# DreamOneX/yet-another-bpe

Measured on AMD Instinct MI355X. Metric: merges_per_sec, higher is better.
Workload: dtype u16

## Files before the change

### yet-another-bpe_amd/csrc/yabpe.hip

```cpp
#include <hip/hip_runtime.h>
#include <dlfcn.h>
#include <rccl/rccl.h>

#include <algorithm>
#include <cstdarg>
#include <cstddef>
#include <cstdio>
#include <cstring>
#include <map>
#include <mutex>
#include <string>
#include <vector>

#include "../../include/yabpe.h"
#include "yabpe_kernels.h"
#include "yabpe_aux_kernels.h"
#include "yabpe_devmem.h"
#include "yabpe_pretok_kernels.h"
#include "yabpe_encode_kernels.h"
#include "yabpe_dropout_kernels.h"
#include "yabpe_decode_kernels.h"
#include "yabpe_layout_kernels.h"
#include "yabpe_replay_kernels.h"
#include "yabpe_pool_kernels.h"
// ... 134 lines not shown
    uint8_t *dec_text = nullptr;
    unsigned long long *dec_doc = nullptr;
    yabpe_decode_stats_t dec_stats{};
    hipEvent_t dec_ev[7] = {};
    uint32_t *lay_buf[7] = {};
    yabpe_layout_stats_t lay_stats{};
    hipEvent_t lay_ev[4] = {};
    yabpe_resume_stats_t resume_stats{};
    bool have_pool = false;
    PoolView wpool{};
    uint64_t wpool_arena_cap = 0, wpool_n = 0, wpool_bytes = 0;
    yabpe_pool_stats_t wpool_stats{};
    hipEvent_t wpool_ev[4] = {};
    unsigned long long *scratch64 = nullptr;
    unsigned long long *blk_stats = nullptr;
    uint32_t blk_used = 0;
    bool split_mode = false;
    uint32_t kmax_now = 1;
    std::vector<float> ev_scan_us;
    unsigned long long *sig = nullptr;
    uint32_t sig_stride = 0;
    unsigned long long *blk_read = nullptr;
    uint64_t scan_skip_launches = 0;
    uint64_t piece_tag = 0;
    bool sig_valid = false;
    uint32_t sig_built_at = 0;
    uint64_t sig_tokens_at_build = 0;
    uint64_t sig_builds = 0;
    CandState *cand_state = nullptr;
    uint32_t cand_built_at = 0;
    unsigned long long cand_best_at_build = 0;
    uint32_t *sel_ticket = nullptr;
    unsigned long long *cand = nullptr;
    bool use_cand = false;
    uint64_t cand_rebuilds = 0, cand_rescans = 0;
    double cand_margin = 0.2;
    uint32_t cand_n_at_build = 0;
    bool pending = false;
    uint64_t fused_launches = 0;
    int rank = 0, n_ranks = 1;
    bool multi = false;
    ncclComm_t comm = nullptr;
    yabpe_allgather_fn ag_fn = nullptr;
    void *ag_user = nullptr;
    unsigned long long *xsmall = nullptr;
    uint8_t *xsend = nullptr, *xrecv = nullptr;
    uint64_t exchange_growths = 0;
    uint64_t exchange_max_records = 0;
    uint32_t xcap = 0;
    uint64_t xstride = 0;
    uint32_t xeff = 0;
    uint64_t xeff_sum = 0;
    uint32_t xseen[4] = {0, 0, 0, 0};
    uint64_t exchanges = 0;
    bool p2p = false;
    uint8_t *p2p_area = nullptr;
    std::vector<uint8_t *> p2p_peer;
    uint64_t p2p_half = 0, p2p_flags_off = 0, p2p_seq = 0, p2p_stride = 0;
    uint32_t p2p_cap = 0;
    hipEvent_t p2p_e0 = nullptr, p2p_e1 = nullptr;
    bool p2p_pending = false;
    int id_bits = 16;
    bool id_bits_fixed = false;
    uint32_t *tiles32 = nullptr, *tiles32_alt = nullptr, *long_tok32 = nullptr;
    uint32_t tiles32_alt_cap = 0;
    PairTable32 table32{};
// ... 69 lines not shown

int fill_u16(yabpe_ctx *c, uint16_t *p, uint64_t n, uint16_t v) {
    if (!n) return 0;
    uint64_t th = (n + 7) / 8;
    hipLaunchKernelGGL(k_fill_u16, dim3(cdiv64(th, 256)), dim3(256), 0, c->stream, p, (unsigned long long)n, v);
    HIPCHK(c, hipGetLastError());
    return 0;
}
int fill_u32(yabpe_ctx *c, uint32_t *p, uint64_t n, uint32_t v) {
    if (!n) return 0;
    hipLaunchKernelGGL(k_fill_u32, dim3(cdiv64(n, 256)), dim3(256), 0, c->stream, p, (unsigned long long)n, v);
    HIPCHK(c, hipGetLastError());
    return 0;
}

int state_pull(yabpe_ctx *c) {
    HIPCHK(c, hipMemcpyAsync(c->st_host, c->st, sizeof(DevState), hipMemcpyDeviceToHost, c->stream));
    HIPCHK(c, hipStreamSynchronize(c->stream));
    return 0;
}
int state_push(yabpe_ctx *c) {
    HIPCHK(c, hipMemcpyAsync(c->st, c->st_host, sizeof(DevState), hipMemcpyHostToDevice, c->stream));
    HIPCHK(c, hipStreamSynchronize(c->stream));
    return 0;
}

void table_free(PairTable &t) {
    dfree(t.keys);
    dfree(t.cnt);
    t.keys = nullptr;
    t.cnt = nullptr;
    t.cand_cs = nullptr;
    t.cand_list = nullptr;
    t.cand_T = 0;
    t.sink_rec = nullptr;
    t.sink_hdr = nullptr;
    t.sink_cap = 0;
}

int table_alloc(yabpe_ctx *c, PairTable &t, uint64_t cap, unsigned long long *entries_ctr) {
    TRY(dmalloc(c, &t.keys, cap));
    TRY(dmalloc(c, &t.cnt, cap));
    t.cap = (uint32_t)cap;
    t.max_probe = c->multi ? (uint32_t)cap : (uint32_t)std::min<uint64_t>(cap, 2048);
    t.sink_rec = nullptr;
    t.sink_hdr = nullptr;
    t.sink_cap = 0;
    t.entries = entries_ctr;
    t.cand_cs = nullptr;
    t.cand_list = nullptr;
    t.cand_T = 0;
    HIPCHK(c, hipMemsetAsync(t.keys, 0xFF, cap * sizeof(uint32_t), c->stream));
    HIPCHK(c, hipMemsetAsync(t.cnt, 0, cap * sizeof(unsigned long long), c->stream));
    return 0;
}

int cand_attach(yabpe_ctx *c) {
    c->use_cand = false;
    PairTable &t = c->table;
    t.cand_cs = nullptr;
    t.cand_list = nullptr;
    if (!optv(c, "cand_argmax", 1)) return 0;
    if (!c->sel_ticket) {
        TRY(dmalloc(c, &c->sel_ticket, TICKET_WORDS));
        HIPCHK(c, hipMemsetAsync(c->sel_ticket, 0, TICKET_WORDS * 4, c->stream));
    }
    if (!c->cand_state) {
        TRY(dmalloc(c, &c->cand_state, 1));
        TRY(dmalloc(c, &c->cand, CAND_CAP));
    }
    return 0;
}

int cand_rebuild(yabpe_ctx *c, unsigned long long best_count) {
    c->use_cand = false;
    c->table.cand_cs = nullptr;
    c->table.cand_list = nullptr;
    if (!optv(c, "cand_argmax", 1) || !c->cand_state || best_count < (unsigned long long)optv(c, "cand_min_count", 16)) return 0;
    const uint32_t target = (uint32_t)std::max<int64_t>(64, optv(c, "cand_target", 768));
    const uint32_t grid = (uint32_t)std::min<uint64_t>(1024, std::max<uint64_t>(1, c->table_cap / (BLOCK * 8)));
    CandState h{};
    for (int attempt = 0; attempt < 12; ++attempt) {
        unsigned long long margin = (unsigned long long)((double)best_count * c->cand_margin);
        if (margin < 1) margin = 1;
        h = CandState{best_count - std::min(margin, best_count - 1), 0u, 0u, 0u, 0u};
        HIPCHK(c, hipMemcpyAsync(c->cand_state, &h, sizeof h, hipMemcpyHostToDevice, c->stream));
        PairTable t = c->table;
        t.cand_list = c->cand;
        t.cand_cs = c->cand_state;
        t.cand_T = h.T;
        {
            CandParams P{t, c->tt.rec, c->partials, c->st, c->cand_state, nullptr, SelectParams{}};
            hipLaunchKernelGGL(k_cand_rebuild, dim3(grid), dim3(BLOCK), 0, c->stream, P);
        }
        HIPCHK(c, hipGetLastError());
        HIPCHK(c, hipMemcpyAsync(&h, c->cand_state, sizeof h, hipMemcpyDeviceToHost, c->stream));
        HIPCHK(c, hipStreamSynchronize(c->stream));
        c->cand_rebuilds++;
        if ((h.overflow || h.n > target) && margin > 1) {
            c->cand_margin *= 0.5;
            continue;
        }
        break;
    }
    if (h.n < target / 8) c->cand_margin = std::min((double)optv(c, "cand_margin_max_pct", 60) / 100.0, c->cand_margin * 2.0);
    c->use_cand = !h.overflow && h.n < CAND_CAP / 2;
    c->cand_n_at_build = h.n;
    if (c->use_cand) {
        c->table.cand_cs = c->cand_state;
        c->table.cand_list = c->cand;
        c->table.cand_T = h.T;
    }
    return 0;
}

uint32_t count_grid(yabpe_ctx *c) {
    return count_grid_rule(c->n_tiles, (uint32_t)c->n_cu, (uint32_t)c->apply_occ, optv(c, "apply_blocks", OPT_UNSET));
}

int fold_stats(yabpe_ctx *c) {
    FoldParams F{c->st, c->blk_stats, std::max(c->blk_used, 1u)};
    hipLaunchKernelGGL(k_fold_stats, dim3(1), dim3(BLOCK), 0, c->stream, F);
    HIPCHK(c, hipGetLastError());
    c->blk_used = 0;
    return 0;
}

int comm_allgather(yabpe_ctx *c, const void *send, void *recv, uint64_t nbytes) {
    if (c->comm) {
        NCCLCHK(c, rccl()->AllGather(send, recv, nbytes, ncclUint8, c->comm, c->stream));
        return 0;
    }
    if (!c->ag_fn) return fail(c, YABPE_E_COMM, "no transport attached");
    HIPCHK(c, hipStreamSynchronize(c->stream));
    int rc = c->ag_fn(c->ag_user, send, recv, nbytes);
    if (rc != 0) return fail(c, YABPE_E_COMM, "custom all-gather transport failed (%d)", rc);
    return 0;
}

int comm_max(yabpe_ctx *c, unsigned long long v, unsigned long long *out);

int exchange_table(yabpe_ctx *c, PairTable lt, uint64_t lcap, PairTable t) {
    unsigned long long *d_cnt = &c->scratch64[8];
// ... 737 lines not shown
    for (auto &e : c->enc_ev)
        if (e) (void)hipEventDestroy(e);
    yabpe_decode_free(c);
    dfree(c->dec_ent); dfree(c->dec_pool);
    for (auto &e : c->dec_ev)
        if (e) (void)hipEventDestroy(e);
    yabpe_layout_free(c);
    for (auto &e : c->lay_ev)
        if (e) (void)hipEventDestroy(e);
    yabpe_pool_clear(c);
    for (auto &e : c->wpool_ev)
        if (e) (void)hipEventDestroy(e);
    dfree(c->pt_cls);
    dfree(c->pt_cls5);
    yabpe_normalize_free(c);
    dfree(c->nfc_prop); dfree(c->nfc_decomp); dfree(c->nfc_pairs);
    for (auto &e : c->norm_ev)
        if (e) (void)hipEventDestroy(e);
    free_corpus(c);
    id32_free_corpus(c);
    dfree(c->partials32);
    dfree(c->cand32_state);
    dfree(c->cand32_list);
    free_records(c);
    dfree(c->tt.pool); dfree(c->tt.off); dfree(c->tt.len); dfree(c->tt.rec); dfree(c->tt.vset);
    dfree(c->partials);
    dfree(c->st);
    dfree(c->scratch64);
    dfree(c->blk_stats);
    dfree(c->blk_read);
    dfree(c->cand_state);
    dfree(c->sel_ticket);
    dfree(c->cand);
    dfree(c->xsend);
    dfree(c->xrecv);
    dfree(c->xsmall);
    p2p_close(c);
    if (c->p2p_e0) (void)hipEventDestroy(c->p2p_e0);
    if (c->p2p_e1) (void)hipEventDestroy(c->p2p_e1);
    if (c->comm && rccl()) (void)rccl()->CommDestroy(c->comm);
    if (c->st_host) (void)hipHostFree(c->st_host);
    for (auto &e : c->events) {
        (void)hipEventDestroy(e.e0);
        (void)hipEventDestroy(e.e1);
        (void)hipEventDestroy(e.e2);
    }
    if (c->stream) (void)hipStreamDestroy(c->stream);
    delete c;
}

int yabpe_set_option(yabpe_ctx *c, const char *name, int64_t value) {
    if (!c || !name) return YABPE_E_INVALID;
    if (strcmp(name, "id_bits") == 0) {
        if (value != 16 && value != 32) return fail(c, YABPE_E_INVALID, "option id_bits is %lld: 16 or 32", (long long)value);
        if (c->id_bits_fixed && value != c->id_bits)
            return fail(c, YABPE_E_INVALID, "option id_bits cannot change after yabpe_set_vocab (it is %d)", c->id_bits);
        if (value == 32 && c->multi) return fail(c, YABPE_E_INVALID, "id_bits = 32 is single-device: this context has a communicator attached");
        if (!c->id_bits_fixed) c->id_bits = (int)value;
    }
    c->opt[name] = value;
    return YABPE_OK;
}

int yabpe_set_vocab(yabpe_ctx *c, const uint8_t *tok_bytes, const uint32_t *tok_off, uint32_t n_tokens) {
    if (!c) return YABPE_E_INVALID;
    HIPCHK(c, hipSetDevice(c->device));
// ... 2740 lines not shown
```

### yet-another-bpe_amd/csrc/yabpe_kernels.h

```cpp
#pragma once
#include <hip/hip_runtime.h>
#include <stdint.h>

#include <type_traits>

#include "limit_logic.h"
#include "load_logic.h"
#include "steal_logic.h"
#include "tile_logic.h"
#include "train_rules.h"

namespace yb {

constexpr int CAP = 1024;
constexpr int LMAX = 64;
constexpr int SPAN = CAP - LMAX + 1;
constexpr uint32_t EMPTY = 0xFFFFFFFFu;
constexpr uint32_t PADPAD = (YB_PAD << 16) | YB_PAD;
constexpr int LONG_CH = 1024;
constexpr int SIG_ROWS = 512;
constexpr int SIG_ROWS_LOG2 = 9;
constexpr int SIG_TILES = 8;
constexpr int MAX_LISTS_PROF = 4096;
constexpr int SCAN_CHUNK = 256;
constexpr int SCAN_KT_MAX = 4;

enum : uint32_t { HALT_NONE = 0, HALT_TABLE_FULL = 1, HALT_POOL_FULL = 2, HALT_VOCAB_FULL = 3, HALT_DELTA_FULL = 4, HALT_RESCAN = 5, HALT_COMM = 6 };

struct BatchMerge {
    uint32_t a, b, c, is_new;
};
struct DevState {
    uint32_t iter;
    uint32_t done;
    uint32_t halt;
    uint32_t halt_req;
    uint32_t a, b, c;
    uint32_t c_is_new;
    uint32_t n_tokens;
    uint32_t pool_used;
// ... 13 lines not shown
    uint32_t n_batch;
    uint32_t n_select;
    BatchMerge batch[KMAX];
    const uint32_t *tok_len;
    uint32_t max_token_bytes;
    uint32_t pad_limit;
};

struct DeltaHdr {
    unsigned long long count;
    unsigned long long halt;
};
struct DeltaRec {
    uint32_t key, pad;
    long long delta;
};

constexpr uint32_t CAND_CAP = 1u << 16;
struct CandState {
    unsigned long long T;
    uint32_t n, overflow;
    uint32_t n_seen;
    uint32_t pad;
};

struct PairTable {
    uint32_t *keys;
    unsigned long long *cnt;
    uint32_t cap;
    uint32_t max_probe;
    unsigned long long *entries;
    CandState *cand_cs;
    unsigned long long *cand_list;
    unsigned long long cand_T;
    DeltaRec *sink_rec;
    DeltaHdr *sink_hdr;
    uint32_t sink_cap;
};
__device__ __forceinline__ uint32_t hash32(uint32_t k);
__device__ __forceinline__ uint32_t pt_home(const PairTable &t, uint32_t key) {
    return (uint32_t)(((unsigned long long)hash32(key) * t.cap) >> 32);
}
__device__ __forceinline__ uint32_t pt_next(const PairTable &t, uint32_t s) { return s + 1 == t.cap ? 0u : s + 1; }

struct Best {
    unsigned long long cnt;
    uint32_t rk;
    uint32_t key;
    uint32_t slot;
    uint32_t pad;
};

__device__ __forceinline__ void best_store_coherent(Best *p, const Best &b) {
    unsigned long long *q = reinterpret_cast<unsigned long long *>(p);
    __hip_atomic_store(q + 0, b.cnt, __ATOMIC_RELAXED, __HIP_MEMORY_SCOPE_AGENT);
    __hip_atomic_store(q + 1, ((unsigned long long)b.key << 32) | b.rk, __ATOMIC_RELAXED, __HIP_MEMORY_SCOPE_AGENT);
    __hip_atomic_store(q + 2, (unsigned long long)b.slot, __ATOMIC_RELAXED, __HIP_MEMORY_SCOPE_AGENT);
}
__device__ __forceinline__ Best best_load_coherent(const Best *p) {
    unsigned long long *q = reinterpret_cast<unsigned long long *>(const_cast<Best *>(p));
    const unsigned long long a = __hip_atomic_load(q + 0, __ATOMIC_RELAXED, __HIP_MEMORY_SCOPE_AGENT);
    const unsigned long long b = __hip_atomic_load(q + 1, __ATOMIC_RELAXED, __HIP_MEMORY_SCOPE_AGENT);
    const unsigned long long c = __hip_atomic_load(q + 2, __ATOMIC_RELAXED, __HIP_MEMORY_SCOPE_AGENT);
    return Best{a, (uint32_t)b, (uint32_t)(b >> 32), (uint32_t)c, 0u};
}

// ... 38 lines not shown
    const SigHash H = sig_hash(key);
    return SigProbe{sig + (size_t)H.row * stride, H.mask};
}

__device__ __forceinline__ void vm_drain() { __builtin_amdgcn_s_waitcnt(0x0F70); }

__device__ __forceinline__ void wave_sync() {
    __builtin_amdgcn_fence(__ATOMIC_RELEASE, "wavefront");
    __builtin_amdgcn_wave_barrier();
    __builtin_amdgcn_fence(__ATOMIC_ACQUIRE, "wavefront");
}

__device__ __forceinline__ unsigned long long lanemask_lt(int lane) { return (1ull << lane) - 1ull; }
__device__ __forceinline__ uint32_t bits_below_lane(unsigned long long m) {
    return __builtin_amdgcn_mbcnt_hi((uint32_t)(m >> 32), __builtin_amdgcn_mbcnt_lo((uint32_t)m, 0u));
}

__device__ __forceinline__ uint32_t wave_inclusive_sum(uint32_t x) {
    x += (uint32_t)__builtin_amdgcn_update_dpp(0, (int)x, 0x111, 0xf, 0xf, true);
    x += (uint32_t)__builtin_amdgcn_update_dpp(0, (int)x, 0x112, 0xf, 0xf, true);
    x += (uint32_t)__builtin_amdgcn_update_dpp(0, (int)x, 0x114, 0xf, 0xf, true);
    x += (uint32_t)__builtin_amdgcn_update_dpp(0, (int)x, 0x118, 0xf, 0xf, true);
    x += (uint32_t)__builtin_amdgcn_update_dpp(0, (int)x, 0x142, 0xa, 0xf, false);
    x += (uint32_t)__builtin_amdgcn_update_dpp(0, (int)x, 0x143, 0xc, 0xf, false);
    return x;
}

__device__ __forceinline__ void st_coherent(unsigned long long *p, unsigned long long v) { __hip_atomic_store(p, v, __ATOMIC_RELAXED, __HIP_MEMORY_SCOPE_AGENT); }
__device__ __forceinline__ void st_coherent(uint32_t *p, uint32_t v) { __hip_atomic_store(p, v, __ATOMIC_RELAXED, __HIP_MEMORY_SCOPE_AGENT); }
__device__ __forceinline__ unsigned long long ld_coherent(const unsigned long long *p) { return __hip_atomic_load(const_cast<unsigned long long *>(p), __ATOMIC_RELAXED, __HIP_MEMORY_SCOPE_AGENT); }
__device__ __forceinline__ uint32_t ld_coherent(const uint32_t *p) { return __hip_atomic_load(const_cast<uint32_t *>(p), __ATOMIC_RELAXED, __HIP_MEMORY_SCOPE_AGENT); }

__device__ __forceinline__ void cand_note(const PairTable &t, uint32_t s, uint32_t key, unsigned long long old, unsigned long long now) {
    if ((long long)now < (long long)t.cand_T || (long long)old >= (long long)t.cand_T || (long long)now <= 0) return;
    const uint32_t idx = atomicAdd(&t.cand_cs->n, 1u);
    if (idx < CAND_CAP)
        st_coherent(&t.cand_list[idx], (unsigned long long)s | ((unsigned long long)key << 32));
    else
        st_coherent(&t.cand_cs->overflow, 1u);
}
__device__ __forceinline__ unsigned long long *pt_count_ptr(const PairTable &t, unsigned long long entry) { return &t.cnt[(uint32_t)entry]; }
__device__ __forceinline__ void gt_bump(const PairTable &t, uint32_t s, uint32_t key, long long d) {
    if (d > 0 && t.cand_list) {
        const unsigned long long old = atomicAdd(&t.cnt[s], (unsigned long long)d);
        cand_note(t, s, key, old, old + (unsigned long long)d);
    } else {
        atomicAdd(&t.cnt[s], (unsigned long long)d);
    }
}

__device__ __forceinline__ void sink_append(const PairTable &t, uint32_t key, long long d) {
    const unsigned long long idx = atomicAdd(&t.sink_hdr->count, 1ull);
    if (idx < t.sink_cap) t.sink_rec[idx] = DeltaRec{key, 0u, d};
}
__device__ __forceinline__ void gt_add_from(const PairTable &t, DevState *st, uint32_t key, long long d, uint32_t s, uint32_t *inserted) {
    if (t.sink_rec) {
        sink_append(t, key, d);
        return;
    }
    for (uint32_t probe = 0; probe < t.max_probe; ++probe) {
        uint32_t k = __hip_atomic_load(&t.keys[s], __ATOMIC_RELAXED, __HIP_MEMORY_SCOPE_AGENT);
        if (k == EMPTY) {
            const uint32_t lim = st->max_token_bytes;
            if (lim != 0u) {
                const uint32_t *len = st->tok_len;
                if (!yb_pair_fits(len[key >> 16], len[key & 0xffffu], lim)) return;
            }
// ... 1685 lines not shown
    __syncthreads();
    if ((tid & 63) == 0) {
        s_b[tid >> 6] = best;
        if (fa | ff) {
            atomicAdd(&s_fold[0], fa);
            atomicAdd(&s_fold[1], ff);
        }
    }
    __syncthreads();
    YB_SEL_STAMP(2);
    if (tid == 0) {
        for (int w = 1; w < WPB; ++w)
            if (best_gt(s_b[w], best)) best = s_b[w];
        s_flag = sel_stop(P, S, s_fold[0], s_fold[1], best.cnt);
        s_m.cnt = best.cnt;
        s_m.key = best.key;
        s_m.slot = best.slot;
    }
    __syncthreads();
    if (s_flag) return;
    YB_SEL_STAMP(3);
    if (tid < 2) {
        const TokRec r = P.tt.rec[tid ? s_m.key & 0xffffu : s_m.key >> 16];
        if (tid) { s_m.hy = r.hash; s_m.ly = r.len; s_m.py = r.pre8; } else { s_m.hx = r.hash; s_m.lx = r.len; s_m.px = r.pre8; }
    }
    __syncthreads();
    YB_SEL_STAMP(4);
    if (tid < 64) commit_merge(P, S, s_m);
    YB_SEL_STAMP(7);
}

__device__ __forceinline__ void select_eval(const SelectParams &P, WinEnt *s_win) {
    __shared__ AccEnt s_acc[KMAX];
    __shared__ __attribute__((aligned(16))) uint32_t s_hset[2 * WIN];
    __shared__ unsigned long long s_red[WPB], s_fold[2];
    __shared__ uint32_t s_nwin;
    struct TopEnt { unsigned long long cnt; uint32_t key, win; };
    __shared__ unsigned long long s_lim[2];
    __shared__ uint32_t s_flags[2];
    unsigned long long *s_pk = reinterpret_cast<unsigned long long *>(s_hset);
    __shared__ TopEnt s_top[KMAX];
    static_assert(BLOCK == 2 * WIN, "two threads rank one window entry");
    constexpr uint32_t HSET = 2 * WIN;
    DevState *st = P.st;
    const int tid = threadIdx.x;
    const int lane = tid & 63;
    YB_SEL_STAMP(1);
    unsigned long long e[4], cn[4];
#pragma unroll
    for (int k = 0; k < 4; ++k) e[k] = ld_coherent(&P.table.cand_list[tid + k * BLOCK]);
    const uint32_t n_list = min(ld_coherent(&P.cs->n), CAND_CAP);
    const uint32_t kmax = min(st->kmax, (uint32_t)KMAX);
    SelState S{};
    if (tid == 0) {
        S = sel_state_load(P, true);
        s_fold[0] = 0;
        s_fold[1] = 0;
        s_nwin = 0;
        s_flags[0] = 0u;
        s_flags[1] = 0u;
        s_lim[0] = S.candT;
        s_lim[1] = S.min_freq;
    }
    unsigned long long vx[4], vy[4];
#pragma unroll
    for (int k = 0; k < 4; ++k) {
        const uint32_t i = k * BLOCK + tid;
        vx[k] = i < P.n_blk ? ld_coherent(&P.blk_stats[2 * i]) : 0ull;
        vy[k] = i < P.n_blk ? ld_coherent(&P.blk_stats[2 * i + 1]) : 0ull;
    }
    for (uint32_t hidx = tid; hidx < HSET; hidx += BLOCK) s_hset[hidx] = EMPTY;
#pragma unroll
    for (int k = 0; k < 4; ++k) {
        cn[k] = 0ull;
        if ((uint32_t)(tid + k * BLOCK) < n_list) cn[k] = ld_coherent(pt_count_ptr(P.table, e[k]));
    }
    unsigned long long fa = 0, ff = 0;
    {
        unsigned long long *bs = P.blk_stats;
#pragma unroll
        for (int k = 0; k < 4; ++k) {
            const uint32_t i = k * BLOCK + tid;
            fa += vx[k];
            ff += vy[k];
            if (i < P.n_blk && (vx[k] | vy[k])) {
                bs[2 * i] = 0ull;
                bs[2 * i + 1] = 0ull;
            }
        }
        for (uint32_t i = 4 * BLOCK + tid; i < P.n_blk; i += BLOCK) {
            const unsigned long long x = ld_coherent(&bs[2 * i]), y = ld_coherent(&bs[2 * i + 1]);
            fa += x;
            ff += y;
            if (x | y) {
                bs[2 * i] = 0ull;
                bs[2 * i + 1] = 0ull;
            }
        }
    }
    fa = wave_sum_u64(fa);
    ff = wave_sum_u64(ff);
    YB_SEL_STAMP(9);
    unsigned long long cmax = 0ull;
#pragma unroll
    for (int k = 0; k < 4; ++k) {
        if ((long long)cn[k] <= 0) cn[k] = 0ull;
        cmax = cn[k] > cmax ? cn[k] : cmax;
    }
    for (uint32_t ti = 4u * BLOCK + tid; ti < n_list; ti += BLOCK) {
        const long long c = (long long)ld_coherent(pt_count_ptr(P.table, ld_coherent(&P.table.cand_list[ti])));
        if (c > 0 && (unsigned long long)c > cmax) cmax = (unsigned long long)c;
    }
    YB_SEL_STAMP(10);
    cmax = best_wave_reduce(Best{cmax, 0u, 0u, 0u, 0u}).cnt;
    __syncthreads();
    if (lane == 0) {
        s_red[tid >> 6] = cmax;
        if (fa | ff) {
            atomicAdd(&s_fold[0], fa);
            atomicAdd(&s_fold[1], ff);
        }
    }
    __syncthreads();
#pragma unroll
    for (int w = 0; w < WPB; ++w) cmax = s_red[w] > cmax ? s_red[w] : cmax;
    YB_SEL_STAMP(12);
    unsigned long long L = 0ull;
    uint32_t n_win = 0;
    uint32_t wshift = min(max(st->win_shift, 1u), 20u), narrowed = 0;
    if (cmax) {
        unsigned long long delta = kmax > 1u ? min(max((unsigned long long)kmax, cmax >> wshift), 1ull << 31) : 0ull;
        for (int attempt = 0; attempt < 8; ++attempt) {
            L = cmax > delta ? cmax - delta : 1ull;
            if (kmax > 1u && L < s_lim[0] && cmax >= s_lim[0]) L = s_lim[0];
            auto put = [&](unsigned long long ent, unsigned long long c) {
                const uint32_t key = (uint32_t)(ent >> 32);
                uint32_t h = hash32(key) & (HSET - 1u);
                for (uint32_t probe = 0; probe < HSET; ++probe) {
                    const uint32_t was = atomicCAS(&s_hset[h], EMPTY, key);
                    if (was == key) return;
                    if (was == EMPTY) {
                        const uint32_t idx = atomicAdd(&s_nwin, 1u);
                        if (idx < (uint32_t)WIN) {
                            s_win[idx].cnt = c;
                            s_win[idx].key = key;
                            s_win[idx].slot = (uint32_t)ent;
                        }
                        return;
                    }
                    h = (h + 1u) & (HSET - 1u);
                }
                s_nwin = WIN + 1u;
            };
#pragma unroll
            for (int k = 0; k < 4; ++k)
                if (cn[k] >= L) put(e[k], cn[k]);
            for (uint32_t ti = 4u * BLOCK + tid; ti < n_list; ti += BLOCK) {
                const unsigned long long ent = ld_coherent(&P.table.cand_list[ti]);
                const long long c = (long long)ld_coherent(pt_count_ptr(P.table, ent));
                if (c > 0 && (unsigned long long)c >= L) put(ent, (unsigned long long)c);
            }
            __syncthreads();
            n_win = s_nwin;
            if (n_win <= (uint32_t)WIN) break;
            n_win = 0;
            if (delta == 0ull) break;
            delta >>= 2;
            narrowed += 2;
            __syncthreads();
            for (uint32_t hidx = tid; hidx < HSET; hidx += BLOCK) s_hset[hidx] = EMPTY;
            if (tid == 0) s_nwin = 0;
            __syncthreads();
        }
    }
    if (cmax && n_win == 0) {
        __shared__ Best s_tb[WPB];
        Best tb{0ull, 0u, EMPTY, 0u, 0u};
        auto consider = [&](unsigned long long ent) {
            const uint32_t key = (uint32_t)(ent >> 32);
            const uint32_t rl = (uint32_t)ld_coherent(reinterpret_cast<const unsigned long long *>(&P.tt.rec[key >> 16]));
            const uint32_t rr = (uint32_t)ld_coherent(reinterpret_cast<const unsigned long long *>(&P.tt.rec[key & 0xffffu]));
            const Best b{1ull, (rl << 16) | rr, key, (uint32_t)ent, 0u};
            if (best_gt(b, tb)) tb = b;
        };
#pragma unroll 1
        for (int k = 0; k < 4; ++k)
            if (cn[k] == cmax) consider(e[k]);
        for (uint32_t ti = 4u * BLOCK + tid; ti < n_list; ti += BLOCK) {
            const unsigned long long ent = ld_coherent(&P.table.cand_list[ti]);
            if (ld_coherent(pt_count_ptr(P.table, ent)) == cmax) consider(ent);
        }
        tb = best_wave_reduce(tb);
        __syncthreads();
        if (lane == 0) s_tb[tid >> 6] = tb;
        __syncthreads();
        if (tid == 0) {
            for (int w = 1; w < WPB; ++w)
                if (best_gt(s_tb[w], tb)) tb = s_tb[w];
            s_win[0].cnt = cmax;
            s_win[0].key = tb.key;
            s_win[0].slot = tb.slot;
        }
        __syncthreads();
        n_win = 1;
    }
    YB_SEL_STAMP(13);
    if ((uint32_t)tid < n_win) {
        const uint32_t key = s_win[tid].key;
        const unsigned long long *qx = reinterpret_cast<const unsigned long long *>(&P.tt.rec[key >> 16]);
        const unsigned long long *qy = reinterpret_cast<const unsigned long long *>(&P.tt.rec[key & 0xffffu]);
        const unsigned long long ax = ld_coherent(qx), hx = ld_coherent(qx + 1), px = ld_coherent(qx + 2);
        const unsigned long long ay = ld_coherent(qy), hy = ld_coherent(qy + 1), py = ld_coherent(qy + 2);
        s_win[tid].rk = ((uint32_t)ax << 16) | ((uint32_t)ay & 0xffffu);
        s_win[tid].lx = (uint32_t)(ax >> 32);
        s_win[tid].ly = (uint32_t)(ay >> 32);
        s_win[tid].hx = hx;
        s_win[tid].hy = hy;
        s_win[tid].px = px;
        s_win[tid].py = py;
        s_pk[tid] = ((s_win[tid].cnt - L) << 32) | (unsigned long long)(((uint32_t)ax << 16) | ((uint32_t)ay & 0xffffu));
    } else if (tid < WIN) {
        s_pk[tid] = 0ull;
    }
    __syncthreads();
    YB_SEL_STAMP(11);
    const uint32_t wt = (uint32_t)(tid >> 6) * 32u + ((uint32_t)lane & 31u), whalf = (uint32_t)lane >> 5;
    uint32_t my_pos = 0xffffu, my_key = 0u;
    unsigned long long my_cnt = 0ull;
    {
        const unsigned long long mine = s_pk[wt];
        const ulonglong2 *pk2 = reinterpret_cast<const ulonglong2 *>(s_pk) + whalf * (uint32_t)(WIN / 4);
        uint32_t above = 0;
#pragma unroll 8
        for (uint32_t m = 0; m < (uint32_t)(WIN / 4); ++m) {
            const ulonglong2 kk = pk2[m];
            above += (kk.x > mine ? 1u : 0u) + (kk.y > mine ? 1u : 0u);
        }
        above += __shfl_xor(above, 32);
        if (whalf == 0u && wt < n_win) {
            my_pos = above;
            my_key = s_win[wt].key;
            my_cnt = s_win[wt].cnt;
            if (my_pos < (uint32_t)KMAX) {
                s_top[my_pos] = TopEnt{my_cnt, my_key, wt};
                s_acc[my_pos] = AccEnt{my_key >> 16, my_key & 0xffffu, s_win[wt].lx + s_win[wt].ly, wt, pre8_concat(s_win[wt].px, s_win[wt].lx, s_win[wt].py)};
            }
        }
    }
    __syncthreads();
    const uint32_t n_top = min(n_win, (uint32_t)KMAX);
    if (my_pos != 0xffffu) {
        const uint32_t topmask = (1u << n_top) - 1u;
        uint32_t ra = 0, lb = 0, tie = 0;
#pragma unroll
        for (uint32_t i2 = 0; i2 < (uint32_t)KMAX; ++i2) {
            const TopEnt te = s_top[i2];
            ra |= (uint32_t)((my_key & 0xffffu) == (te.key >> 16)) << i2;
            lb |= (uint32_t)((my_key >> 16) == (te.key & 0xffffu)) << i2;
            tie |= (uint32_t)(te.cnt == my_cnt) << i2;
        }
        ra &= topmask;
        lb &= topmask;
        if (my_pos < (uint32_t)KMAX) {
            const uint32_t below = (1u << my_pos) - 1u;
            if (my_pos != 0u && (((ra | lb) & below) != 0u || my_cnt < s_lim[0] || my_cnt < s_lim[1])) atomicOr(&s_flags[0], 1u << my_pos);
            if ((my_key >> 16) == (my_key & 0xffffu)) atomicOr(&s_flags[1], 1u << my_pos);
        }
        const uint32_t touch = ra | lb;
        uint32_t cand = touch ? tie & topmask & ~((2u << (__ffs((int)touch) - 1)) - 1u) & (my_pos < (uint32_t)KMAX ? (1u << my_pos) - 1u : ~0u) : 0u;
        for (; cand; cand &= cand - 1u) {
            const uint32_t j2 = (uint32_t)__ffs((int)cand) - 1u, below = (1u << j2) - 1u;
            const uint32_t cwin = s_top[j2].win;
            const unsigned long long c_px = s_win[cwin].px, c_py = s_win[cwin].py;
            const uint32_t c_lx = s_win[cwin].lx, c_ly = s_win[cwin].ly;
            bool left_new_blocks = false, right_new_ge = false;
            for (uint32_t m = lb & below; m; m &= m - 1u) {
                const AccEnt A = s_acc[__ffs((int)m) - 1];
                left_new_blocks |= cmp_pre8(A.pc, A.lc, c_px, c_lx) != -1;
            }
            for (uint32_t m = ra & below; m; m &= m - 1u) {
                const AccEnt A = s_acc[__ffs((int)m) - 1];
                right_new_ge |= cmp_pre8(A.pc, A.lc, c_py, c_ly) != -1;
            }
            const uint32_t rl = s_win[wt].rk >> 16, rp = s_win[cwin].rk >> 16;
            if (left_new_blocks || ((ra & below) != 0u && (rl > rp || (rl == rp && right_new_ge)))) atomicOr(&s_flags[0], 1u << j2);
        }
    }
    __syncthreads();
    YB_SEL_STAMP(14);
    if (tid >= 64) return;
    uint32_t flag = 0;
    if (lane == 0) {
        flag = sel_stop(P, S, s_fold[0], s_fold[1], cmax);
        if (kmax > 1u) st->win_shift = narrowed ? min(wshift + narrowed, 20u) : (n_win < 4u * kmax && wshift > 1u) ? wshift - 1u : wshift;
    }
    flag = __builtin_amdgcn_readfirstlane(flag);
    if (flag) return;
    YB_SEL_STAMP(3);
    const uint32_t it0 = __builtin_amdgcn_readfirstlane(S.iter), num_merges = __builtin_amdgcn_readfirstlane(S.num_merges);
    uint32_t nacc = min(min(kmax, num_merges - it0), n_top), why = 4u;
    (void)why;
    {
        const uint32_t fails = s_flags[0] & ~1u, runs = s_flags[1];
        if (nacc == n_top && n_top < kmax && n_top < num_merges - it0) why = 5u;
        if (fails && (uint32_t)(__ffs((int)fails) - 1) < nacc) {
            nacc = (uint32_t)(__ffs((int)fails) - 1);
            why = 1u;
        }
        if (runs && (uint32_t)__ffs((int)runs) < nacc) {
            nacc = (uint32_t)__ffs((int)runs);
            why = 6u;
        }
    }
    YB_STOP(it0, why, nacc, n_win);
    unsigned long long Hk = 0ull, ve = VSET_EMPTY;
    uint32_t Lk = 0, vslot = 0, wk = 0;
    if ((uint32_t)lane < nacc) {
        wk = s_acc[lane].win;
        const uint32_t lxk = s_win[wk].lx, lyk = s_win[wk].ly;
        Lk = lxk + lyk;
        Hk = yb_hash_concat(s_win[wk].hx, s_win[wk].hy, lyk);
        vslot = yb_vset_home(Hk, Lk) & P.tt.vset_mask;
        ve = ld_coherent(&P.tt.vset[vslot]);
        while (ve != VSET_EMPTY && (ve >> 32) != (Hk >> 32)) {
            vslot = (vslot + 1) & P.tt.vset_mask;
            ve = ld_coherent(&P.tt.vset[vslot]);
        }
    }
    YB_SEL_STAMP(5);
    const bool hit = (uint32_t)lane < nacc && ve != VSET_EMPTY;
    uint32_t bad = hit ? 1u : 0u;
    for (uint32_t k2 = 0; k2 + 1 < nacc; ++k2) {
        const uint32_t s2 = __builtin_amdgcn_readlane(vslot, k2), l2 = __builtin_amdgcn_readlane(Lk, k2);
        const unsigned long long h2 = ((unsigned long long)__builtin_amdgcn_readlane((uint32_t)(Hk >> 32), k2) << 32) | __builtin_amdgcn_readlane((uint32_t)Hk, k2);
        if ((uint32_t)lane < nacc && (uint32_t)lane > k2 && (s2 == vslot || (h2 == Hk && l2 == Lk))) bad = 1u;
    }
    const uint32_t ntok0 = __builtin_amdgcn_readfirstlane(S.n_tokens), pool0 = __builtin_amdgcn_readfirstlane(S.pool_used);
    uint32_t pool_at = pool0;
    for (uint32_t k2 = 0; k2 + 1 < nacc; ++k2) {
        const uint32_t l2 = __builtin_amdgcn_readlane(Lk, k2);
        if ((uint32_t)lane > k2) pool_at += (l2 + 3u) & ~3u;
    }
    if ((uint32_t)lane < nacc && (ntok0 + (uint32_t)lane >= YB_MAX_TOKENS || (unsigned long long)pool_at + Lk + 4ull > P.tt.pool_cap)) bad = 1u;
    const unsigned long long badm = __ballot(bad != 0u);
    const uint32_t keep = badm ? (uint32_t)(__ffsll((long long)badm) - 1) : nacc;
    unsigned long long others_sum = 0ull;
    {
        const unsigned long long mycnt = (uint32_t)lane + 1u < keep ? s_win[wk].cnt : 0ull;
        others_sum = wave_sum_u64(mycnt);
    }
    if ((uint32_t)lane < keep) {
        const uint32_t k = (uint32_t)lane;
        const uint32_t cid = ntok0 + k, key = s_win[wk].key;
        P.tt.off[cid] = pool_at;
        P.tt.len[cid] = Lk;
        P.tt.rec[cid] = TokRec{0u, Lk, Hk, s_acc[k].pc, 0ull};
// ... 292 lines not shown
    if (threadIdx.x >= BLOCK) return;
    YB_SEL_STAMP(8);
    select_eval(F.sel, win);
}

__global__ __launch_bounds__(BLOCK) void k_argmax_cand(CandParams P) {
    __shared__ Best s_b[WPB];
#ifdef YB_PROFILE_SCAN
    if (blockIdx.x == 0) YB_SEL_STAMP(0);
    if (blockIdx.x == 0) YB_SEL_STAMP(8);
#endif
    const uint32_t stop = P.st->done | P.st->halt;
    if (!stop) {
        Best best = cand_list_best(P.table, P.rec, min(P.cs->n, CAND_CAP), blockIdx.x * BLOCK + threadIdx.x, gridDim.x * BLOCK);
        best = best_wave_reduce(best);
        const int lane = threadIdx.x & 63, wib = threadIdx.x >> 6;
        if (lane == 0) s_b[wib] = best;
        __syncthreads();
        if (threadIdx.x == 0) {
            for (int i = 1; i < WPB; ++i)
                if (best_gt(s_b[i], best)) best = s_b[i];
            best_store_coherent(&P.partials[blockIdx.x], best);
        }
#ifdef YB_PROFILE_SCAN
        if (blockIdx.x == 0) YB_SEL_STAMP(9);
#endif
    }
    if (!last_workgroup(P.ticket)) return;
    select_body(P.sel);
}

__global__ __launch_bounds__(BLOCK) void k_cand_rebuild(CandParams P) {
    const unsigned long long T = P.cs->T;
    for (uint32_t s = blockIdx.x * BLOCK + threadIdx.x; s < P.table.cap; s += gridDim.x * BLOCK) {
        const long long cn = (long long)P.table.cnt[s];
        if (cn <= 0 || (unsigned long long)cn < T) continue;
        const uint32_t idx = atomicAdd(&P.cs->n, 1u);
        if (idx < CAND_CAP) P.table.cand_list[idx] = (unsigned long long)s | ((unsigned long long)P.table.keys[s] << 32); else P.cs->overflow = 1u;
    }
}

struct BatchLds {
    uint32_t a[KMAX], b[KMAX], c[KMAX];
    uint32_t row[KMAX];
    unsigned long long mask[KMAX];
};

template <bool WEIGHTED, bool HIST = false>
__global__ __launch_bounds__(BLOCK) void k_apply(ApplyParams P, uint32_t apply_blocks, RankParams R, FuseParams F, LongParams LW, uint32_t long_first) {
    using AggV = typename std::conditional<WEIGHTED, unsigned long long, int>::type;
    static_assert(!(HIST && WEIGHTED), "the direct-indexed store holds 32-bit deltas");
    __shared__ uint32_t s_keys[HIST ? 1 : AGG_N];
    __shared__ AggV s_vals[HIST ? 1 : AGG_N];
    __shared__ int s_hist[HIST ? 4 * HIST_V : 1];
    __shared__ __attribute__((aligned(16))) WaveLds s_w[WPB];
    __shared__ unsigned long long s_cnt[2];

    DevState *st = P.st;
    if (st->done | st->halt) return;
    if (blockIdx.x >= long_first) {
        apply_long_block(LW, blockIdx.x - long_first);
    } else if (blockIdx.x >= apply_blocks) {
        rank_update_block(R, blockIdx.x - apply_blocks);
    } else {
    const int lane = threadIdx.x & 63;
    const int wib = __builtin_amdgcn_readfirstlane(threadIdx.x >> 6);
    SlowCtx<AggV> C{P, Agg<AggV>{s_keys, s_vals, HIST ? 0u : (uint32_t)AGG_N - 1u}, st, st->a, st->b, st->c, 0u, 0u, lane,
                    KeyMemo{{EMPTY, EMPTY, EMPTY, EMPTY}, {0u, 0u, 0u, 0u}}, HIST ? s_hist : nullptr};
    C.mk = yb_memkey(C.a, C.b);
    C.self = yb_pairkey(C.a, C.b);
    const uint32_t mk = C.mk;
// ... 575 lines not shown
```

Measured before the change: 49560.

## Deduplicate candidate list with bitmap and use wave-ballot window compaction in select

Adds a per-slot candidate bitmap so each table slot enters the candidate list at most once. This lets the select kernel drop its shared-memory hash set and compact window entries with wave ballots plus a single atomic per wave. The rebuild kernel now fills the bitmap and appends entries with wave-aggregated atomics. Select also starts loading its state on a separate wave, computes the stop flag earlier, and prefetches vset probe entries during ranking so the final wave has less latency to wait on. The cost is an extra atomicOr on every threshold crossing in the apply path and extra device memory for the bitmap.

```diff
diff --git a/yet-another-bpe_amd/csrc/select_logic.h b/yet-another-bpe_amd/csrc/select_logic.h
--- /dev/null
+++ b/yet-another-bpe_amd/csrc/select_logic.h
@@ -0,0 +1,53 @@
+#pragma once
+#include <stdint.h>
+
+#include "tile_logic.h"
+
+#define YB_WIN_ATTEMPTS 8
+
+YB_HD bool yb_cand_crosses(unsigned long long old, unsigned long long now, unsigned long long T) {
+    return (long long)now >= (long long)T && (long long)old < (long long)T && (long long)now > 0;
+}
+YB_HD uint64_t yb_cand_bitmap_words(uint64_t table_cap) { return (table_cap + 63u) / 64u; }
+YB_HD uint32_t yb_cand_word(uint32_t slot) { return slot >> 6; }
+YB_HD unsigned long long yb_cand_bit(uint32_t slot) { return 1ull << (slot & 63u); }
+YB_HD bool yb_cand_lists(unsigned long long word_before, uint32_t slot) { return (word_before & yb_cand_bit(slot)) == 0ull; }
+YB_HD bool yb_cand_rebuild_lists(unsigned long long count, unsigned long long T) { return (long long)count > 0 && count >= T; }
+
+YB_HD unsigned long long yb_win_delta0(uint32_t kmax, unsigned long long cmax, uint32_t wshift) {
+    if (kmax <= 1u) return 0ull;
+    unsigned long long d = cmax >> wshift;
+    if (d < (unsigned long long)kmax) d = (unsigned long long)kmax;
+    return d < (1ull << 31) ? d : (1ull << 31);
+}
+YB_HD unsigned long long yb_win_floor(unsigned long long cmax, unsigned long long delta, uint32_t kmax, unsigned long long T) {
+    unsigned long long L = cmax > delta ? cmax - delta : 1ull;
+    if (kmax > 1u && L < T && cmax >= T) L = T;
+    return L;
+}
+YB_HD unsigned long long yb_win_narrow(unsigned long long delta) { return delta >> 2; }
+
+struct YbWindow {
+    unsigned long long L;
+    uint32_t n;
+    uint32_t narrowed;
+};
+template <class CountF>
+YB_HD YbWindow yb_win_search(unsigned long long cmax, uint32_t kmax, uint32_t wshift, unsigned long long T, uint32_t win, CountF count) {
+    YbWindow w{0ull, 0u, 0u};
+    if (!cmax) return w;
+    unsigned long long delta = yb_win_delta0(kmax, cmax, wshift);
+    for (int attempt = 0; attempt < YB_WIN_ATTEMPTS; ++attempt) {
+        w.L = yb_win_floor(cmax, delta, kmax, T);
+        const uint32_t n = count(w.L, attempt);
+        if (n <= win) {
+            w.n = n;
+            break;
+        }
+        if (delta == 0ull) break;
+        delta = yb_win_narrow(delta);
+        w.narrowed += 2u;
+    }
+    return w;
+}
+YB_HD bool yb_win_fallback(unsigned long long cmax, const YbWindow &w) { return cmax != 0ull && w.n == 0u; }
diff --git a/yet-another-bpe_amd/csrc/yabpe.hip b/yet-another-bpe_amd/csrc/yabpe.hip
--- a/yet-another-bpe_amd/csrc/yabpe.hip
+++ b/yet-another-bpe_amd/csrc/yabpe.hip
@@ -190,6 +190,8 @@
     unsigned long long cand_best_at_build = 0;
     uint32_t *sel_ticket = nullptr;
     unsigned long long *cand = nullptr;
+    unsigned long long *cand_bits = nullptr;
+    uint64_t cand_bits_cap = 0;
     bool use_cand = false;
     uint64_t cand_rebuilds = 0, cand_rescans = 0;
     double cand_margin = 0.2;
@@ -325,6 +327,7 @@
     t.cnt = nullptr;
     t.cand_cs = nullptr;
     t.cand_list = nullptr;
+    t.cand_bits = nullptr;
     t.cand_T = 0;
     t.sink_rec = nullptr;
     t.sink_hdr = nullptr;
@@ -342,6 +345,7 @@
     t.entries = entries_ctr;
     t.cand_cs = nullptr;
     t.cand_list = nullptr;
+    t.cand_bits = nullptr;
     t.cand_T = 0;
     HIPCHK(c, hipMemsetAsync(t.keys, 0xFF, cap * sizeof(uint32_t), c->stream));
     HIPCHK(c, hipMemsetAsync(t.cnt, 0, cap * sizeof(unsigned long long), c->stream));
@@ -353,6 +357,10 @@
     PairTable &t = c->table;
     t.cand_cs = nullptr;
     t.cand_list = nullptr;
+    t.cand_bits = nullptr;
+    dfree(c->cand_bits);
+    c->cand_bits = nullptr;
+    c->cand_bits_cap = 0;
     if (!optv(c, "cand_argmax", 1)) return 0;
     if (!c->sel_ticket) {
         TRY(dmalloc(c, &c->sel_ticket, TICKET_WORDS));
@@ -369,7 +377,15 @@
     c->use_cand = false;
     c->table.cand_cs = nullptr;
     c->table.cand_list = nullptr;
+    c->table.cand_bits = nullptr;
     if (!optv(c, "cand_argmax", 1) || !c->cand_state || best_count < (unsigned long long)optv(c, "cand_min_count", 16)) return 0;
+    if (!c->cand_bits || c->cand_bits_cap != c->table.cap) {
+        dfree(c->cand_bits);
+        c->cand_bits = nullptr;
+        c->cand_bits_cap = 0;
+        TRY(dmalloc(c, &c->cand_bits, yb_cand_bitmap_words(c->table.cap)));
+        c->cand_bits_cap = c->table.cap;
+    }
     const uint32_t target = (uint32_t)std::max<int64_t>(64, optv(c, "cand_target", 768));
     const uint32_t grid = (uint32_t)std::min<uint64_t>(1024, std::max<uint64_t>(1, c->table_cap / (BLOCK * 8)));
     CandState h{};
@@ -380,6 +396,7 @@
         HIPCHK(c, hipMemcpyAsync(c->cand_state, &h, sizeof h, hipMemcpyHostToDevice, c->stream));
         PairTable t = c->table;
         t.cand_list = c->cand;
+        t.cand_bits = c->cand_bits;
         t.cand_cs = c->cand_state;
         t.cand_T = h.T;
         {
@@ -402,6 +419,7 @@
     if (c->use_cand) {
         c->table.cand_cs = c->cand_state;
         c->table.cand_list = c->cand;
+        c->table.cand_bits = c->cand_bits;
         c->table.cand_T = h.T;
     }
     return 0;
@@ -1205,6 +1223,7 @@
     dfree(c->cand_state);
     dfree(c->sel_ticket);
     dfree(c->cand);
+    dfree(c->cand_bits);
     dfree(c->xsend);
     dfree(c->xrecv);
     dfree(c->xsmall);
diff --git a/yet-another-bpe_amd/csrc/yabpe_kernels.h b/yet-another-bpe_amd/csrc/yabpe_kernels.h
--- a/yet-another-bpe_amd/csrc/yabpe_kernels.h
+++ b/yet-another-bpe_amd/csrc/yabpe_kernels.h
@@ -6,6 +6,7 @@
 
 #include "limit_logic.h"
 #include "load_logic.h"
+#include "select_logic.h"
 #include "steal_logic.h"
 #include "tile_logic.h"
 #include "train_rules.h"
@@ -85,6 +86,7 @@
     unsigned long long *entries;
     CandState *cand_cs;
     unsigned long long *cand_list;
+    unsigned long long *cand_bits;
     unsigned long long cand_T;
     DeltaRec *sink_rec;
     DeltaHdr *sink_hdr;
@@ -189,7 +191,8 @@
 __device__ __forceinline__ uint32_t ld_coherent(const uint32_t *p) { return __hip_atomic_load(const_cast<uint32_t *>(p), __ATOMIC_RELAXED, __HIP_MEMORY_SCOPE_AGENT); }
 
 __device__ __forceinline__ void cand_note(const PairTable &t, uint32_t s, uint32_t key, unsigned long long old, unsigned long long now) {
-    if ((long long)now < (long long)t.cand_T || (long long)old >= (long long)t.cand_T || (long long)now <= 0) return;
+    if (!yb_cand_crosses(old, now, t.cand_T)) return;
+    if (!yb_cand_lists(atomicOr(&t.cand_bits[yb_cand_word(s)], yb_cand_bit(s)), s)) return;
     const uint32_t idx = atomicAdd(&t.cand_cs->n, 1u);
     if (idx < CAND_CAP)
         st_coherent(&t.cand_list[idx], (unsigned long long)s | ((unsigned long long)key << 32));
@@ -1941,16 +1944,19 @@
 
 __device__ __forceinline__ void select_eval(const SelectParams &P, WinEnt *s_win) {
     __shared__ AccEnt s_acc[KMAX];
-    __shared__ __attribute__((aligned(16))) uint32_t s_hset[2 * WIN];
+    __shared__ __attribute__((aligned(16))) unsigned long long s_pk[WIN];
     __shared__ unsigned long long s_red[WPB], s_fold[2];
     __shared__ uint32_t s_nwin;
     struct TopEnt { unsigned long long cnt; uint32_t key, win; };
+    struct ProbeEnt { unsigned long long H, ve; uint32_t slot, len; };
+    struct StopEnt { unsigned long long live_slots; uint32_t flag, iter, num_merges, n_tokens, pool_used, pad; };
     __shared__ unsigned long long s_lim[2];
     __shared__ uint32_t s_flags[2];
-    unsigned long long *s_pk = reinterpret_cast<unsigned long long *>(s_hset);
     __shared__ TopEnt s_top[KMAX];
+    __shared__ ProbeEnt s_probe[KMAX];
+    __shared__ StopEnt s_stop;
     static_assert(BLOCK == 2 * WIN, "two threads rank one window entry");
-    constexpr uint32_t HSET = 2 * WIN;
+    constexpr int S_TID = BLOCK - 64;
     DevState *st = P.st;
     const int tid = threadIdx.x;
     const int lane = tid & 63;
@@ -1962,12 +1968,14 @@
     const uint32_t kmax = min(st->kmax, (uint32_t)KMAX);
     SelState S{};
     if (tid == 0) {
-        S = sel_state_load(P, true);
         s_fold[0] = 0;
         s_fold[1] = 0;
         s_nwin = 0;
         s_flags[0] = 0u;
         s_flags[1] = 0u;
+    }
+    if (tid == S_TID) {
+        S = sel_state_load(P, true);
         s_lim[0] = S.candT;
         s_lim[1] = S.min_freq;
     }
@@ -1978,11 +1986,11 @@
         vx[k] = i < P.n_blk ? ld_coherent(&P.blk_stats[2 * i]) : 0ull;
         vy[k] = i < P.n_blk ? ld_coherent(&P.blk_stats[2 * i + 1]) : 0ull;
     }
-    for (uint32_t hidx = tid; hidx < HSET; hidx += BLOCK) s_hset[hidx] = EMPTY;
 #pragma unroll
     for (int k = 0; k < 4; ++k) {
-        cn[k] = 0ull;
-        if ((uint32_t)(tid + k * BLOCK) < n_list) cn[k] = ld_coherent(pt_count_ptr(P.table, e[k]));
+        const bool listed = (uint32_t)(tid + k * BLOCK) < n_list;
+        cn[k] = ld_coherent(pt_count_ptr(P.table, listed ? e[k] : 0ull));
+        if (!listed) cn[k] = 0ull;
     }
     unsigned long long fa = 0, ff = 0;
     {
@@ -2034,54 +2042,55 @@
 #pragma unroll
     for (int w = 0; w < WPB; ++w) cmax = s_red[w] > cmax ? s_red[w] : cmax;
     YB_SEL_STAMP(12);
-    unsigned long long L = 0ull;
-    uint32_t n_win = 0;
-    uint32_t wshift = min(max(st->win_shift, 1u), 20u), narrowed = 0;
-    if (cmax) {
-        unsigned long long delta = kmax > 1u ? min(max((unsigned long long)kmax, cmax >> wshift), 1ull << 31) : 0ull;
-        for (int attempt = 0; attempt < 8; ++attempt) {
-            L = cmax > delta ? cmax - delta : 1ull;
-            if (kmax > 1u && L < s_lim[0] && cmax >= s_lim[0]) L = s_lim[0];
-            auto put = [&](unsigned long long ent, unsigned long long c) {
-                const uint32_t key = (uint32_t)(ent >> 32);
-                uint32_t h = hash32(key) & (HSET - 1u);
-                for (uint32_t probe = 0; probe < HSET; ++probe) {
-                    const uint32_t was = atomicCAS(&s_hset[h], EMPTY, key);
-                    if (was == key) return;
-                    if (was == EMPTY) {
-                        const uint32_t idx = atomicAdd(&s_nwin, 1u);
-                        if (idx < (uint32_t)WIN) {
-                            s_win[idx].cnt = c;
-                            s_win[idx].key = key;
-                            s_win[idx].slot = (uint32_t)ent;
-                        }
-                        return;
-                    }
-                    h = (h + 1u) & (HSET - 1u);
-                }
-                s_nwin = WIN + 1u;
-            };
-#pragma unroll
-            for (int k = 0; k < 4; ++k)
-                if (cn[k] >= L) put(e[k], cn[k]);
-            for (uint32_t ti = 4u * BLOCK + tid; ti < n_list; ti += BLOCK) {
-                const unsigned long long ent = ld_coherent(&P.table.cand_list[ti]);
-                const long long c = (long long)ld_coherent(pt_count_ptr(P.table, ent));
-                if (c > 0 && (unsigned long long)c >= L) put(ent, (unsigned long long)c);
-            }
+    const uint32_t wshift = min(max(st->win_shift, 1u), 20u);
+    const YbWindow wnd = yb_win_search(cmax, kmax, wshift, s_lim[0], (uint32_t)WIN, [&](unsigned long long Lf, int attempt) -> uint32_t {
+        if (attempt) {
             __syncthreads();
-            n_win = s_nwin;
-            if (n_win <= (uint32_t)WIN) break;
-            n_win = 0;
-            if (delta == 0ull) break;
-            delta >>= 2;
-            narrowed += 2;
-            __syncthreads();
-            for (uint32_t hidx = tid; hidx < HSET; hidx += BLOCK) s_hset[hidx] = EMPTY;
             if (tid == 0) s_nwin = 0;
             __syncthreads();
         }
-    }
+        auto place = [&](bool in, unsigned long long ent, unsigned long long c, unsigned long long b, uint32_t at) {
+            const uint32_t idx = at + bits_below_lane(b);
+            if (in && idx < (uint32_t)WIN) {
+                s_win[idx].cnt = c;
+                s_win[idx].key = (uint32_t)(ent >> 32);
+                s_win[idx].slot = (uint32_t)ent;
+            }
+        };
+        unsigned long long b[4];
+        uint32_t tot = 0, at = 0;
+#pragma unroll
+        for (int k = 0; k < 4; ++k) {
+            b[k] = __ballot(cn[k] >= Lf);
+            tot += (uint32_t)__popcll(b[k]);
+        }
+        if (lane == 0 && tot) at = atomicAdd(&s_nwin, tot);
+        at = __builtin_amdgcn_readfirstlane(at);
+#pragma unroll
+        for (int k = 0; k < 4; ++k) {
+            place(cn[k] >= Lf, e[k], cn[k], b[k], at);
+            at += (uint32_t)__popcll(b[k]);
+        }
+        for (uint32_t t0 = 4u * BLOCK + (uint32_t)(tid & ~63); t0 < n_list; t0 += BLOCK) {
+            const uint32_t ti = t0 + (uint32_t)lane;
+            unsigned long long ent = 0ull;
+            long long c = 0;
+            if (ti < n_list) {
+                ent = ld_coherent(&P.table.cand_list[ti]);
+                c = (long long)ld_coherent(pt_count_ptr(P.table, ent));
+            }
+            const bool in = c > 0 && (unsigned long long)c >= Lf;
+            const unsigned long long bb = __ballot(in);
+            uint32_t at2 = 0;
+            if (lane == 0 && bb) at2 = atomicAdd(&s_nwin, (uint32_t)__popcll(bb));
+            place(in, ent, (unsigned long long)c, bb, __builtin_amdgcn_readfirstlane(at2));
+        }
+        __syncthreads();
+        return s_nwin;
+    });
+    const unsigned long long L = wnd.L;
+    const uint32_t narrowed = wnd.narrowed;
+    uint32_t n_win = wnd.n;
     if (cmax && n_win == 0) {
         __shared__ Best s_tb[WPB];
         Best tb{0ull, 0u, EMPTY, 0u, 0u};
@@ -2114,6 +2123,15 @@
         n_win = 1;
     }
     YB_SEL_STAMP(13);
+    if (tid == S_TID) {
+        s_stop.flag = sel_stop(P, S, s_fold[0], s_fold[1], cmax);
+        s_stop.iter = S.iter;
+        s_stop.num_merges = S.num_merges;
+        s_stop.n_tokens = S.n_tokens;
+        s_stop.pool_used = S.pool_used;
+        s_stop.live_slots = S.live_slots;
+        if (kmax > 1u) st->win_shift = narrowed ? min(wshift + narrowed, 20u) : (n_win < 4u * kmax && wshift > 1u) ? wshift - 1u : wshift;
+    }
     if ((uint32_t)tid < n_win) {
         const uint32_t key = s_win[tid].key;
         const unsigned long long *qx = reinterpret_cast<const unsigned long long *>(&P.tt.rec[key >> 16]);
@@ -2136,6 +2154,7 @@
     const uint32_t wt = (uint32_t)(tid >> 6) * 32u + ((uint32_t)lane & 31u), whalf = (uint32_t)lane >> 5;
     uint32_t my_pos = 0xffffu, my_key = 0u;
     unsigned long long my_cnt = 0ull;
+    ProbeEnt my_probe{0ull, VSET_EMPTY, 0u, 0u};
     {
         const unsigned long long mine = s_pk[wt];
         const ulonglong2 *pk2 = reinterpret_cast<const ulonglong2 *>(s_pk) + whalf * (uint32_t)(WIN / 4);
@@ -2151,8 +2170,15 @@
             my_key = s_win[wt].key;
             my_cnt = s_win[wt].cnt;
             if (my_pos < (uint32_t)KMAX) {
+                const WinEnt &w = s_win[wt];
+                const uint32_t lx = w.lx, ly = w.ly;
+                const unsigned long long px = w.px, py = w.py;
                 s_top[my_pos] = TopEnt{my_cnt, my_key, wt};
-                s_acc[my_pos] = AccEnt{my_key >> 16, my_key & 0xffffu, s_win[wt].lx + s_win[wt].ly, wt, pre8_concat(s_win[wt].px, s_win[wt].lx, s_win[wt].py)};
+                s_acc[my_pos] = AccEnt{my_key >> 16, my_key & 0xffffu, lx + ly, wt, pre8_concat(px, lx, py)};
+                my_probe.len = lx + ly;
+                my_probe.H = yb_hash_concat(w.hx, w.hy, ly);
+                my_probe.slot = yb_vset_home(my_probe.H, my_probe.len) & P.tt.vset_mask;
+                my_probe.ve = ld_coherent(&P.tt.vset[my_probe.slot]);
             }
         }
     }
@@ -2194,17 +2220,17 @@
             const uint32_t rl = s_win[wt].rk >> 16, rp = s_win[cwin].rk >> 16;
             if (left_new_blocks || ((ra & below) != 0u && (rl > rp || (rl == rp && right_new_ge)))) atomicOr(&s_flags[0], 1u << j2);
         }
+        if (my_pos < (uint32_t)KMAX) s_probe[my_pos] = my_probe;
     }
     __syncthreads();
     YB_SEL_STAMP(14);
     if (tid >= 64) return;
-    uint32_t flag = 0;
-    if (lane == 0) {
-        flag = sel_stop(P, S, s_fold[0], s_fold[1], cmax);
-        if (kmax > 1u) st->win_shift = narrowed ? min(wshift + narrowed, 20u) : (n_win < 4u * kmax && wshift > 1u) ? wshift - 1u : wshift;
-    }
-    flag = __builtin_amdgcn_readfirstlane(flag);
-    if (flag) return;
+    if (__builtin_amdgcn_readfirstlane(s_stop.flag)) return;
+    S.iter = s_stop.iter;
+    S.num_merges = s_stop.num_merges;
+    S.n_tokens = s_stop.n_tokens;
+    S.pool_used = s_stop.pool_used;
+    S.live_slots = s_stop.live_slots;
     YB_SEL_STAMP(3);
     const uint32_t it0 = __builtin_amdgcn_readfirstlane(S.iter), num_merges = __builtin_amdgcn_readfirstlane(S.num_merges);
     uint32_t nacc = min(min(kmax, num_merges - it0), n_top), why = 4u;
@@ -2226,11 +2252,11 @@
     uint32_t Lk = 0, vslot = 0, wk = 0;
     if ((uint32_t)lane < nacc) {
         wk = s_acc[lane].win;
-        const uint32_t lxk = s_win[wk].lx, lyk = s_win[wk].ly;
-        Lk = lxk + lyk;
-        Hk = yb_hash_concat(s_win[wk].hx, s_win[wk].hy, lyk);
-        vslot = yb_vset_home(Hk, Lk) & P.tt.vset_mask;
-        ve = ld_coherent(&P.tt.vset[vslot]);
+        const ProbeEnt pe = s_probe[lane];
+        Lk = pe.len;
+        Hk = pe.H;
+        vslot = pe.slot;
+        ve = pe.ve;
         while (ve != VSET_EMPTY && (ve >> 32) != (Hk >> 32)) {
             vslot = (vslot + 1) & P.tt.vset_mask;
             ve = ld_coherent(&P.tt.vset[vslot]);
@@ -2589,11 +2615,21 @@
 
 __global__ __launch_bounds__(BLOCK) void k_cand_rebuild(CandParams P) {
     const unsigned long long T = P.cs->T;
-    for (uint32_t s = blockIdx.x * BLOCK + threadIdx.x; s < P.table.cap; s += gridDim.x * BLOCK) {
-        const long long cn = (long long)P.table.cnt[s];
-        if (cn <= 0 || (unsigned long long)cn < T) continue;
-        const uint32_t idx = atomicAdd(&P.cs->n, 1u);
-        if (idx < CAND_CAP) P.table.cand_list[idx] = (unsigned long long)s | ((unsigned long long)P.table.keys[s] << 32); else P.cs->overflow = 1u;
+    const uint32_t lane = threadIdx.x & 63u;
+    for (unsigned long long s0 = (unsigned long long)blockIdx.x * BLOCK + (threadIdx.x & ~63u); s0 < P.table.cap; s0 += (unsigned long long)gridDim.x * BLOCK) {
+        const uint32_t s = (uint32_t)s0 + lane;
+        const bool lists = s0 + lane < P.table.cap && yb_cand_rebuild_lists(P.table.cnt[s], T);
+        const unsigned long long word = __ballot(lists);
+        uint32_t base = 0;
+        if (lane == 0) {
+            P.table.cand_bits[yb_cand_word((uint32_t)s0)] = word;
+            if (word) base = atomicAdd(&P.cs->n, (uint32_t)__popcll(word));
+        }
+        base = __builtin_amdgcn_readfirstlane(base);
+        if (lists) {
+            const uint32_t idx = base + bits_below_lane(word);
+            if (idx < CAND_CAP) P.table.cand_list[idx] = (unsigned long long)s | ((unsigned long long)P.table.keys[s] << 32); else P.cs->overflow = 1u;
+        }
     }
 }
 
```

Result: faster. 50770 (median of 6 runs) (+2.4%).
